# viridityzhu/HiFiHR

Measured on AMD Instinct MI355X. Metric: train images/sec, FreiHAND 224x224 (ResNet-18 + MANO LBS + render + losses + Adam), higher is better.
Workload: dtype f32; 1 GPU; BASELINE configs[1]: FreiHAND batch=32/GPU, ResNet-18 encoder + MANO LBS + silhouette/texture render losses, 224x224, aa=3 (672^2 samples); per_gpu_batch=32, global_batch=32, parallelism=dp1

## Files before the change

### hifihr_amd/_lib.py

```python
from __future__ import annotations

import ctypes
import os
from ctypes import POINTER, c_char_p, c_float, c_int, c_int32, c_long, c_size_t, c_void_p

import torch

_HERE = os.path.dirname(os.path.abspath(__file__))
LIB_PATH = os.path.join(_HERE, "libhifihr.so")

_c_float_p = POINTER(c_float)


class _LinearDesc(ctypes.Structure):
    _fields_ = [("x", c_void_p), ("w", c_void_p), ("b", c_void_p), ("y", c_void_p), ("B", c_int), ("I", c_int), ("O", c_int), ("act", c_int),
                ("dy", c_void_p), ("dz_scratch", c_void_p), ("dW_acc", c_void_p), ("db_acc", c_void_p), ("dx", c_void_p)]

_c_int_p = POINTER(c_int32)


class HifihrError(RuntimeError):
    pass


# ... 114 lines not shown
        c.hifihr_photo_loss_partial_floats.restype = c_int
        c.hifihr_photo_loss_fwd.argtypes = [_c_float_p, _c_float_p, c_void_p, c_int, c_int, c_int, c_float, c_float, c_float] + \
            [_c_float_p] * 4 + [c_void_p]
        c.hifihr_photo_loss_bwd.argtypes = [_c_float_p] * 6 + [c_int, c_int, c_int, c_float, c_float, _c_float_p, c_void_p]
        c.hifihr_sil_post.argtypes = [_c_float_p, _c_float_p, c_int, c_int, c_int, _c_float_p, _c_float_p, c_void_p]
        c.hifihr_linear_fwd.argtypes = [_c_float_p] * 3 + [c_int] * 4 + [_c_float_p] * 2 + [c_float, c_float] + [_c_float_p] * 6 + [c_void_p]
        c.hifihr_linear_bwd.argtypes = [_c_float_p] * 4 + [c_int] * 4 + [_c_float_p] * 10 + [c_void_p]
        c.hifihr_linear_fwd_group.argtypes = [POINTER(_LinearDesc), c_int, c_void_p]
        c.hifihr_linear_bwd_group.argtypes = [POINTER(_LinearDesc), c_int, c_void_p]
        c.hifihr_conv2d_bwd_data_pre.argtypes = [_c_float_p] * 3 + [c_int] * 9 + [c_void_p, c_size_t, c_void_p]
        c.hifihr_conv2d_bwd_data_pre_res.argtypes = [_c_float_p] * 4 + [c_int] * 9 + [c_void_p, c_size_t, c_void_p]
        c.hifihr_conv2d_bwd_data_pre_plus1x1.argtypes = [_c_float_p] * 5 + [c_int] * 9 + [c_void_p]
        c.hifihr_conv2d_bwd_data_pre_plus1x1_supported.argtypes = [c_int] * 9
        c.hifihr_conv2d_bwd_weight_plus1x1.argtypes = [_c_float_p] * 5 + [c_int] * 9 + [c_void_p]
        c.hifihr_conv2d_bwd_weight_plus1x1_supported.argtypes = [c_int] * 9
        c.hifihr_weight_prep.argtypes = [c_void_p, c_int, c_int, c_void_p]
        c.hifihr_freihand_augment.argtypes = [c_void_p, c_void_p, _c_int_p, _c_int_p, c_int, c_int, c_int, _c_float_p, _c_float_p, c_void_p]
        c.hifihr_ho3d_workspace_bytes.argtypes = [c_int, c_int]
        c.hifihr_ho3d_workspace_bytes.restype = c_size_t
        c.hifihr_ho3d_batch.argtypes = ([c_void_p, c_void_p] + [_c_float_p] * 3 + [c_int, c_int, _c_int_p, c_int, c_int, c_void_p, c_size_t] +
                                        [_c_float_p] * 5 + [c_void_p])
        c.hifihr_freihand_batch.argtypes = ([c_void_p, c_void_p] + [_c_float_p] * 4 + [c_int, c_int, _c_int_p, c_int, c_int, c_int, _c_float_p,
                                            _c_float_p, c_void_p] + [_c_float_p] * 6 + [c_void_p, c_void_p])
        c.hifihr_freihand_batch_step.argtypes = ([c_void_p, c_void_p] + [_c_float_p] * 4 + [c_int, c_int, _c_int_p, c_int, c_int, c_int, _c_float_p,
                                                 _c_float_p, c_void_p] + [_c_float_p] * 6 + [c_void_p, c_int, c_float] + [_c_float_p] * 4 + [c_void_p])
        c.hifihr_light_split_fwd.argtypes = [_c_float_p, c_int, _c_float_p, _c_float_p, c_void_p]
        c.hifihr_light_split_bwd.argtypes = [_c_float_p, _c_float_p, _c_float_p, c_int, _c_float_p, c_void_p]
        c.hifihr_wino4_bwd_gemm_pair_supported.argtypes = [c_int] * 5
        c.hifihr_wino4_bwd_gemm_pair.argtypes = [_c_float_p] * 6 + [c_int] * 6 + [c_void_p]
        c.hifihr_loss_total_fwd.argtypes = [POINTER(_c_float_p), POINTER(c_int), c_int, _c_float_p, c_void_p]
# ... 460 lines not shown
    def conv2d_bwd_data_pre_res(self, dy, wt, res, dx, N, H, W, C, K, R, S, stride, pad, ws=None):
        wsp, wsb = self._ws(ws)
        self.check(self.c.hifihr_conv2d_bwd_data_pre_res(_fp(dy), _fp(wt), _fp(res), _fp(dx), N, H, W, C, K, R, S, stride, pad, wsp, wsb,
                                                         _stream_of(dy)), "hifihr_conv2d_bwd_data_pre_res")

    def conv2d_bwd_data_pre_plus1x1_supported(self, N, H, W, C, K, R, S, stride, pad):
        return bool(self.c.hifihr_conv2d_bwd_data_pre_plus1x1_supported(int(N), int(H), int(W), int(C), int(K), int(R), int(S), int(stride), int(pad)))

    def conv2d_bwd_data_pre_plus1x1(self, dy, wt, dy2, wt2, dx, N, H, W, C, K, R, S, stride, pad):
        self.check(self.c.hifihr_conv2d_bwd_data_pre_plus1x1(_fp(dy), _fp(wt), _fp(dy2), _fp(wt2), _fp(dx), N, H, W, C, K, R, S, stride, pad,
                                                             _stream_of(dy)), "hifihr_conv2d_bwd_data_pre_plus1x1")

    def conv2d_bwd_weight_plus1x1_supported(self, N, H, W, C, K, R, S, stride, pad):
        return bool(self.c.hifihr_conv2d_bwd_weight_plus1x1_supported(int(N), int(H), int(W), int(C), int(K), int(R), int(S), int(stride), int(pad)))

    def conv2d_bwd_weight_plus1x1(self, x, dy, dw, dy2, dw2, N, H, W, C, K, R, S, stride, pad):
        self.check(self.c.hifihr_conv2d_bwd_weight_plus1x1(_fp(x), _fp(dy), _fp(dw), _fp(dy2), _fp(dw2), N, H, W, C, K, R, S, stride, pad,
                                                           _stream_of(x)), "hifihr_conv2d_bwd_weight_plus1x1")

    @staticmethod
    def prep_jobs(jobs, device):
        import struct
        raw = b"".join(struct.pack("<QQiiii", s.data_ptr(), d.data_ptr(), K, C, RS, kind) for s, d, K, C, RS, kind in jobs)
        return torch.frombuffer(bytearray(raw), dtype=torch.uint8).to(device)

    def weight_prep(self, table, njobs, blocks_per_job=64):
        self.check(self.c.hifihr_weight_prep(c_void_p(table.data_ptr()), njobs, blocks_per_job, _stream_of(table)), "hifihr_weight_prep")

    def freihand_batch(self, img_rgbx, mask, Ks, joints, verts, scales, packed, B, out, root_id=None, image_size=None):
        n, H, W = img_rgbx.shape
# ... 497 lines not shown
```

### hifihr_amd/csrc/conv.hip

```cpp
#include <hip/hip_runtime.h>

#include <cstdio>
#include <cstdlib>

#include "hifihr_internal.h"

namespace hifihr {

#if defined(HIFIHR_HOSTSIM)
typedef hs_floatx16 floatx16;
#else
typedef float floatx16 __attribute__((ext_vector_type(16)));
#endif

#if defined(HIFIHR_HOSTSIM)
#define HIFIHR_KEEP(x) ((void)0)
#define HIFIHR_SCHED_FENCE() ((void)0)
#else
#define HIFIHR_SCHED_FENCE() __builtin_amdgcn_sched_barrier(0)
#define HIFIHR_KEEP(x) asm volatile("" : "+v"(x))
#endif


struct SkArgs {
// ... 549 lines not shown
    __syncthreads();
  }
#pragma unroll
  for (int i = 0; i < TM; ++i)
#pragma unroll
    for (int j = 0; j < TN; ++j) {
      const int qq = bq0 + wn * (BN / 2) + j * 32 + r31;
#pragma unroll
      for (int e = 0; e < 16; ++e) {
        const int k = bk0 + wm * (BM / 2) + i * 32 + (e & 3) + 8 * (e >> 2) + 4 * half;
        if (k < K && qq < Q) atomicAdd(dw + (size_t)k * Q + qq, acc[i][j][e]);
      }
    }
}

__global__ __launch_bounds__(256) void weight_transpose_kernel(const float* __restrict__ w, float* __restrict__ wt, int K, int RS, int C) {
  const size_t n = (size_t)K * RS * C;
  for (size_t i = (size_t)blockIdx.x * 256 + threadIdx.x; i < n; i += (size_t)gridDim.x * 256) {
    const int k = (int)(i % K);
    const size_t rest = i / K;
    const int rs = (int)(rest % RS);
    const int c = (int)(rest / RS);
    wt[i] = w[((size_t)k * RS + rs) * C + c];
  }
}

__global__ __launch_bounds__(256) void image_to_nhwc4_kernel(const float* __restrict__ img, float4* __restrict__ out, int B, int H, int W,
                                                            int OH, int OW, int pt, int pl, int normalize) {
  const size_t n = (size_t)B * OH * OW, HW = (size_t)H * W;
  for (size_t i = (size_t)blockIdx.x * 256 + threadIdx.x; i < n; i += (size_t)gridDim.x * 256) {
// ... 403 lines not shown
  else snprintf(out, cap, "%s", kWgradKernelName[(int)k]);
}

bool conv_wgrad_plus1x1_supported(const ConvGeom& g) {
  static const int on = env_int("HIFIHR_WGRAD_PLUS1X1", 1);
  return on && !g.dgrad && g.stride >= 2 && g.pad < g.R && g.pad < g.S && g.batch <= 1 && g.IC % 4 == 0 && g.OC % 4 == 0 &&
         g.OH == (g.IH - 1) / g.stride + 1 && g.OW == (g.IW - 1) / g.stride + 1 && plan_wgrad(g, SIZE_MAX).kernel == WgradKernel::tiled;
}
hipError_t launch_conv_wgrad_plus1x1(const ConvGeom& g, const float* x, const float* dy, float* dw, const float* dy2, float* dw2, hipStream_t st) {
  if (!conv_wgrad_plus1x1_supported(g) || dy2 == nullptr || dw2 == nullptr) return hipErrorInvalidValue;
  const long M = (long)g.N * g.OH * g.OW;
  launch_wgrad_tile<64, 64, 16>(g, g.R * g.S * g.IC, M, device_cus() * 8, x, dy, dw, st, dy2, dw2);
  return hipGetLastError();
}

bool conv_wgrad_c3_supported(const ConvGeom& g) { return g.IC == 4 && conv_stem_wgrad_supported(g); }
hipError_t launch_conv_wgrad_c3(const ConvGeom& g, const float* x, const float* dy, float* dw3, void* ws, size_t ws_bytes, hipStream_t st) {
  if (!conv_wgrad_c3_supported(g) || ws == nullptr || ws_bytes < conv_stem_wgrad_slab_bytes()) return hipErrorInvalidValue;
  return launch_conv_stem_wgrad(g, x, dy, dw3, static_cast<float*>(ws), st, 3);
}

hipError_t launch_conv_wgrad(const ConvGeom& g, const float* x, const float* dy, float* dw, void* ws, size_t ws_bytes, hipStream_t st) {
  const long M = (long)g.N * g.OH * g.OW;
  const int Q = g.R * g.S * g.IC;
  if (g.IC % 4 != 0 || g.OC % 4 != 0) return hipErrorInvalidValue;
  const WgradPlan p = plan_wgrad(g, ws != nullptr ? ws_bytes : 0);
  float* slabs = ws_bytes >= p.ws_bytes ? static_cast<float*>(ws) : nullptr;
  hipError_t e = hipErrorNotReady;
  if (p.kernel == WgradKernel::gemm) {
    e = launch_bgemm_tn(dy, x, slabs, g.OC, g.IC, (int)M, 1, p.parts, st);
// ... 46 lines not shown
```

### hifihr_amd/csrc/gemm.hip

```cpp
#include <hip/hip_runtime.h>

#include <cstdio>
#include <cstdlib>
#include <type_traits>

#include "hifihr_internal.h"
#include "lds_dma.h"

namespace hifihr {

template <int BM, int BN>
__global__ __launch_bounds__(256) void bgemm_nt_kernel(BgemmArgs a) {
  constexpr int WM = BM / 2, WN = BN / 2;
  constexpr int TI = WN / 16, TJ = WM / 16;
  constexpr int STAGE = (BM + BN) * 32;
  constexpr int PA = BM / 32, PB = BN / 32;
  __shared__ __attribute__((aligned(1024))) float lds[2 * STAGE];
  const int tid = threadIdx.x, lane = tid & 63, wave = tid >> 6;
  const int wm = wave >> 1, wn = wave & 1;
  const int r = lane & 15, g = lane >> 4;

  int wg = xcd_remap((int)blockIdx.x, (int)gridDim.x);
  const int tiles_pb = a.tiles_m * a.tiles_n;
  const int p = wg / tiles_pb;
// ... 1316 lines not shown
  }
}

__global__ __launch_bounds__(512) void bgemm_tn_rows_kernel(BgemmArgs a, long per) {
  __shared__ __attribute__((aligned(1024))) float lds[4 * kRowsStage];
  tn_rows_body(a, per, lds, (int)blockIdx.x, (int)gridDim.x);
}

__global__ __launch_bounds__(512) void bgemm_nt_tn_pair_kernel(BgemmArgs a, long per_a, int ga, BgemmArgs b, long per_b) {
  __shared__ __attribute__((aligned(1024))) float lds[4 * kRowsStage];
  if ((int)blockIdx.x < ga) nt_rows_body<0>(a, per_a, lds, (int)blockIdx.x, ga);
  else tn_rows_body(b, per_b, lds, (int)blockIdx.x - ga, (int)gridDim.x - ga);
}

constexpr int kUnset = -(1 << 30);
static int gemm_cus() {
  const int v = env_int("HIFIHR_GEMM_CUS", 0);
  return v > 0 ? v : device_cus();
}
struct GemmEnv {
  int rows, tn_rows, tn_split, tn_coherent, tn_skip, pair, conv_rows, conv_rows_pair;
  int cus, loaders, sk, nt_tile, tn_tile, tn_parts;
  bool rows_on() const { return rows && nt_tile == kUnset; }
  bool tn_rows_on() const { return tn_rows && tn_tile == kUnset && tn_parts == kUnset; }
};
static GemmEnv gemm_env() {
  static const GemmEnv once = [] {
    GemmEnv e{};
    e.rows = env_int("HIFIHR_GEMM_ROWS", 1);
    e.tn_rows = env_int("HIFIHR_GEMM_TN_ROWS", 1); e.tn_split = env_int("HIFIHR_GEMM_TN_SPLIT", 1);
    e.tn_coherent = env_int("HIFIHR_GEMM_TN_COHERENT", 1); e.tn_skip = env_int("HIFIHR_GEMM_TN_SKIP", 1);
// ... 378 lines not shown
```

### hifihr_amd/csrc/hifihr_api.hip

```cpp
#include <hip/hip_runtime.h>

#include <algorithm>
#include <array>
#include <cmath>
#include <cstdarg>
#include <cstdio>
#include <cstring>
#include <new>
#include <vector>

#include "../../include/hifihr.h"
#include "hifihr_internal.h"
#include "mano_math.h"

namespace {

thread_local char g_err[512] = "";

int fail(int code, const char* fmt, ...) {
  va_list ap;
  va_start(ap, fmt);
  vsnprintf(g_err, sizeof(g_err), fmt, ap);
  va_end(ap);
  return code;
// ... 717 lines not shown
int hifihr_conv2d_bwd_weight_plus1x1_supported(int N, int H, int W, int C, int K, int R, int S, int stride, int pad) {
  if (!conv_dims_ok(N, H, W, C, K, R, S, stride, pad) || C % 4 || K % 4) return 0;
  const hifihr::ConvGeom g = conv_geom(N, H, W, C, K, R, S, stride, pad);
  return hifihr::conv_wgrad_plus1x1_supported(g) ? 1 : 0;
}

int hifihr_conv2d_bwd_weight_plus1x1(const float* x, const float* dy, float* dw, const float* dy2, float* dw2, int N, int H, int W, int C, int K,
                                     int R, int S, int stride, int pad, void* stream) {
  if (!x || !dy || !dw || !dy2 || !dw2 || !hifihr_conv2d_bwd_weight_plus1x1_supported(N, H, W, C, K, R, S, stride, pad))
    return fail(HIFIHR_EINVAL, "hifihr_conv2d_bwd_weight_plus1x1: bad argument (see hifihr_conv2d_bwd_weight_plus1x1_supported)");
  const hifihr::ConvGeom g = conv_geom(N, H, W, C, K, R, S, stride, pad);
  HIP_TRY(hifihr::launch_conv_wgrad_plus1x1(g, x, dy, dw, dy2, dw2, (hipStream_t)stream));
  return HIFIHR_OK;
}

int hifihr_weight_prep(const hifihr_prep_job* jobs, int njobs, int blocks_per_job, void* stream) {
  static_assert(sizeof(hifihr_prep_job) == sizeof(hifihr::PrepJob), "hifihr_prep_job layout");
  if (!jobs || njobs <= 0 || blocks_per_job <= 0) return fail(HIFIHR_EINVAL, "hifihr_weight_prep: bad argument");
  HIP_TRY(hifihr::launch_weight_prep(reinterpret_cast<const hifihr::PrepJob*>(jobs), njobs, blocks_per_job, (hipStream_t)stream));
  return HIFIHR_OK;
}

int hifihr_conv2d_bwd_weight(const float* x, const float* dy, float* dw, int N, int H, int W, int C, int K, int R, int S,
                             int stride, int pad, void* stream) {
  return hifihr_conv2d_bwd_weight_ws(x, dy, dw, N, H, W, C, K, R, S, stride, pad, nullptr, 0, stream);
}

size_t hifihr_conv2d_wgrad_workspace_bytes(int N, int H, int W, int C, int K, int R, int S, int stride, int pad) {
  if (!conv_dims_ok(N, H, W, C, K, R, S, stride, pad) || C % 4 || K % 4) return 0;
  const hifihr::ConvGeom g = conv_geom(N, H, W, C, K, R, S, stride, pad);
// ... 931 lines not shown
```

### hifihr_amd/csrc/hifihr_internal.h

```cpp
#pragma once
#include <hip/hip_runtime.h>

#include <cstdint>
#include <cstdlib>
#include <stdint.h>

#include "render_math.h"

namespace hifihr {

inline int device_cus() {
  static int cus = 0;
  if (cus == 0) {
    int dev = 0;
    hipDeviceProp_t prop;
    if (hipGetDevice(&dev) == hipSuccess && hipGetDeviceProperties(&prop, dev) == hipSuccess && prop.multiProcessorCount > 0) cus = prop.multiProcessorCount;
  }
  return cus > 0 ? cus : 256;
}

static inline int env_int(const char* name, int unset) {
  const char* e = getenv(name);
  return e ? atoi(e) : unset;
}
// ... 167 lines not shown
                             float* running_mean, float* running_var, hipStream_t st);
hipError_t launch_bn_act_eval(const float* x, const float* running_mean, const float* running_var, const float* gamma, const float* beta,
                              const float* residual, int act, long M, int C, float eps, float* y, hipStream_t st);
hipError_t launch_bn_act_bwd(const float* dy, const float* y, const float* x, const float* save_mean, const float* save_invstd,
                             const float* gamma, const float* beta, int act, long M, int C, float* red, float* dx, float* dres,
                             float* dgamma_acc, float* dbeta_acc, hipStream_t st);
bool bn_relu_maxpool_supported(int N, int H, int W, int C);
hipError_t launch_bn_relu_maxpool_fwd(const float* x, float* stats, const float* gamma, const float* beta, int N, int H, int W, int C,
                                      float eps, float momentum, float* y, unsigned char* tap, float* save_mean, float* save_invstd,
                                      float* running_mean, float* running_var, hipStream_t st);
hipError_t launch_bn_relu_maxpool_bwd(const float* gy, const unsigned char* tap, const float* x, const float* save_mean,
                                      const float* save_invstd, const float* gamma, const float* beta, int N, int H, int W, int C, float* red,
                                      float* dx, float* dgamma_acc, float* dbeta_acc, hipStream_t st, const float* pooled = nullptr);
size_t conv_wgrad_workspace_bytes(const ConvGeom& g);
hipError_t launch_conv_wgrad(const ConvGeom& g, const float* x, const float* dy, float* dw, void* ws, size_t ws_bytes, hipStream_t st);
bool conv_is_gemm(const ConvGeom& g);
bool conv_wgrad_c3_supported(const ConvGeom& g);
hipError_t launch_conv_wgrad_c3(const ConvGeom& g, const float* x, const float* dy, float* dw3, void* ws, size_t ws_bytes, hipStream_t st);
hipError_t launch_weight_transpose(const float* w, float* wt, int K, int RS, int C, hipStream_t st);
hipError_t launch_image_to_nhwc4(const float* img, float* out, int B, int H, int W, int OH, int OW, int pt, int pl, int normalize,
                                 hipStream_t st);

hipError_t launch_image_scale_to_nhwc4(const float* img, float* out, int B, int H, int W, const float* shift3, const float* scale3,
                                       hipStream_t st);
hipError_t launch_maxpool_notap(const float* x, int N, int H, int W, int C, int k, int s, int p, float* y, hipStream_t st);
int lpips_tap_max_channels();
size_t lpips_tap_partial_floats(int B);
hipError_t launch_lpips_tap(const float* f0, const float* f1, const float* w, int B, int HW, int C, int accumulate, float* partial, float* val,
                            hipStream_t st);

// ... 242 lines not shown
```

### hifihr_amd/ops.py

```python
from __future__ import annotations

import math
import os
import threading

import torch

from ._lib import get_lib, require_cuda


import os as _os

_DEBUG_SYNC = _os.environ.get("HIFIHR_DEBUG_SYNC", "0") == "1"


class _Profile:

    def __init__(self):
        self.on = False
        self.events = []
        self.last_render = None
        self.conv_log = []

    def enable(self):
# ... 635 lines not shown

    def end(self):
        self.active = False


_WEIGHT_PREP = _WeightPrep()


class _DeferredDw:

    def __init__(self):
        self.on = os.environ.get("HIFIHR_DEFER_DW", "1") != "0"
        self.active = False
        self.jobs = []
        self.halo = []
        self.pending = set()
        self.early = os.environ.get("HIFIHR_DEFER_EARLY", "1") != "0"
        self.side, self.home, self._streams, self.n_early = None, None, {}, 0

    def wants(self, w, direct):
        if self.side is not None and w.grad is not None and w.grad.data_ptr() in self.pending:
            torch.cuda.current_stream(self.side.device).wait_stream(self.side)
        return (self.on and self.active and direct and not _ASYNC_WGRAD.active and getattr(w, "_hifihr_grad_ready", None) is None
                and (w.grad is None or w.grad.data_ptr() not in self.pending))

    def add(self, dU, parts, tgt, K, C):
        self.jobs.append((dU, int(parts), tgt, int(K), int(C), torch.cuda.current_stream(tgt.device).cuda_stream))
        self.pending.add(tgt.data_ptr())

    def add_halo(self, slabs, nslab, tgt):
        self.halo.append((slabs, int(nslab), tgt, torch.cuda.current_stream(tgt.device).cuda_stream))
        self.pending.add(tgt.data_ptr())

    def clear(self):
        self.jobs.clear(); self.halo.clear(); self.pending.clear()
        if self.side is not None:
            if not torch.cuda.is_current_stream_capturing():
                torch.cuda.current_stream(self.side.device).wait_stream(self.side)
            self.side = None

    def _run(self, jobs, halo):
        lib = get_lib() if (jobs or halo) else None
        if halo:
            PROFILE.bracket("halo_reduce_multi", lambda: lib.conv_halo_wgrad_reduce_multi([h[:3] for h in halo]))
        if jobs:
            PROFILE.bracket("wino_dw_multi", lambda: lib.wino4_dw_transform_multi([j[:5] for j in jobs]))

    def flush(self):
        jobs, self.jobs = self.jobs, []
        halo, self.halo = self.halo, []
        self.pending.clear()
        self._run(jobs, halo)
        if self.side is not None:
            cur = torch.cuda.current_stream(self.side.device)
            cur.wait_stream(self.side)
            if self.home is not None and self.home != cur:
                self.home.wait_stream(self.side)
            self.side = None

    def flush_early(self, device):
        if not (self.early and self.active and self.side is None and (self.jobs or self.halo)):
            return
        cur = torch.cuda.current_stream(device)
        h = cur.cuda_stream
        jobs, halo = [j for j in self.jobs if j[5] == h], [j for j in self.halo if j[3] == h]
        if not (jobs or halo):
            return
        self.jobs, self.halo = [j for j in self.jobs if j[5] != h], [j for j in self.halo if j[3] != h]
        st = self._streams.get(device)
        if st is None:
            st = self._streams[device] = torch.cuda.Stream(device=device)
        st.wait_stream(cur)
        with torch.cuda.stream(st):
            self._run(jobs, halo)
        self.side, self.home, self.n_early = st, cur, self.n_early + 1


_DEFER_DW = _DeferredDw()


class _AsyncWgrad:

    def __init__(self):
        self.active, self.streams, self.refs = False, {}, []

    def stream(self, device):
        s = self.streams.get(device)
        if s is None:
            s = torch.cuda.Stream(device=device)
# ... 179 lines not shown
            PROFILE.bracket("conv_dgrad", lambda: lib.conv3x3_c64_wino(gy, U2, None, False, dx, None, N, H, W))
        return dx, None
    tgt, dw = _grad_target(w, wk, _CL)
    if PROFILE.on:
        PROFILE.conv_log.append((geom, "c64-pair"))
    nslab = lib.conv2d_wgrad_workspace_bytes(*geom)
    if nslab and dw is None and _DEFER_DW.wants(w, True):
        own = _wino_scratch(gy.device, ("c64slabs", w.data_ptr()), (nslab + 3) // 4)
        box = []
        PROFILE.bracket("conv_dgrad", lambda: box.append(lib.conv3x3_c64_bwd_pair_slabs(gy, U2, g_fork, dx, x, own, N, H, W)))
        _DEFER_DW.add_halo(own, box[-1], tgt)
    else:
        slabs = _wgrad_slabs(gy.device, nslab) if nslab else None
        PROFILE.bracket("conv_dgrad", lambda: lib.conv3x3_c64_bwd_pair(gy, U2, g_fork, dx, x, tgt, N, H, W, ws=slabs))
    return dx, dw


def _direct_dgrad(lib, gy, x, wk, w, geom, g_fork, plus1x1):
    dx = torch.empty_like(x, memory_format=_CL)
    ws = _conv_ws(lib, x.device, geom, True)
    if PROFILE.on:
        PROFILE.conv_log.append((geom, "dgrad" if plus1x1 is None else "dgrad+1x1"))
    wt = _WEIGHT_PREP.get(w, wk, 0)
    if plus1x1 is not None:
        assert wt is not None and g_fork is None
        PROFILE.bracket("conv_dgrad", lambda: lib.conv2d_bwd_data_pre_plus1x1(gy, wt, plus1x1[0], plus1x1[1], dx, *geom))
    elif wt is not None and g_fork is not None:
        PROFILE.bracket("conv_dgrad", lambda: lib.conv2d_bwd_data_pre_res(gy, wt, g_fork, dx, *geom, ws=ws))
    elif wt is not None:
        PROFILE.bracket("conv_dgrad", lambda: lib.conv2d_bwd_data_pre(gy, wt, dx, *geom, ws=ws))
# ... 52 lines not shown
            Yt = yt if yt is not None else _wino_scratch(dev, ("Yt", w.data_ptr()) if _ASYNC_WGRAD.active else "Yt", P * T * K)
            if slabs is None:
                slabs = _wino_wgrad_slabs(lib, w, dw is None, _ASYNC_WGRAD.active, dev, N, H, W, C, K, m)
            if PROFILE.on and not paired:
                PROFILE.conv_log.append((("wino", N, H, W, C, K, m), "gemm-tn"))

            def run_w():
                if yt is None:
                    lib.wino_dy_transform(gy, Yt, N, H, W, K, m)
                _wino_wgrad_tail(lib, v_saved, Yt, slabs, tgt, N, H, W, C, K, m, paired)
            go = lambda: PROFILE.bracket("conv_wgrad_wino", run_w)
            keep = (gy, v_saved, Yt, tgt)
        else:
            if PROFILE.on:
                PROFILE.conv_log.append((geom, "wgrad"))
            nslab = lib.conv2d_wgrad_workspace_bytes(*geom)
            go = lambda: PROFILE.bracket("conv_wgrad", lambda: lib.conv2d_bwd_weight(
                x, gy, tgt, *geom, ws=_wgrad_slabs(gy.device, nslab) if nslab else None))
            keep = (gy, x, tgt)
        if _ASYNC_WGRAD.active and dw is None:
            _ASYNC_WGRAD.launch(dev, go, keep)
        else:
            go()
        if dw is None:
            _grad_ready(w)
    if dx is None and g_fork is not None:
        dx = g_fork
    return dx, dw, db


class _Conv2dMFMA(torch.autograd.Function):
    @staticmethod
    def forward(ctx, x, w, stride, pad, want_stats=False, bias=None, relu=False, grad_premasked=False, mask_input_grad=False, fork=False):
# ... 126 lines not shown
            lib = get_lib()
            if lib.conv2d_bwd_data_pre_plus1x1_supported(N, H, W, C, K1, R, S, stride, pad):
                wt1, wt2 = _WEIGHT_PREP.get(ctx.w1, wk1, 0), _WEIGHT_PREP.get(ctx.w2, wk2, 0)
                if wt1 is not None and wt2 is not None:
                    plus = (gy2.contiguous(memory_format=_CL), wt2)
        if plus is not None:
            w_both = (need_w1 and need_w2 and not _ASYNC_WGRAD.active
                      and lib.conv2d_bwd_weight_plus1x1_supported(N, H, W, C, K1, R, S, stride, pad))
            dw1 = dw2 = None
            if w_both:
                gy1c = gy1.contiguous(memory_format=_CL)
                t1, dw1 = _grad_target(ctx.w1, wk1, _CL)
                t2, dw2 = _grad_target(ctx.w2, wk2, _CL)
                if PROFILE.on:
                    PROFILE.conv_log.append((ctx.geom1, "wgrad+1x1"))
                PROFILE.bracket("conv_wgrad", lambda: lib.conv2d_bwd_weight_plus1x1(x, gy1c, t1, plus[0], t2, N, H, W, C, K1, R, S, stride, pad))
                if dw1 is None:
                    _grad_ready(ctx.w1)
                if dw2 is None:
                    _grad_ready(ctx.w2)
            else:
                dw2 = conv(gy2, wk2, ctx.geom2, ctx.w2, False, need_w2)[1]
            dx, dw1b, _ = conv(gy1, wk1, ctx.geom1, ctx.w1, need_x, need_w1 and not w_both, plus1x1=plus)
            return dx, (dw1 if w_both else dw1b), dw2, None
        dx2 = dw2 = dw1 = None
        if gy2 is not None:
            dx2, dw2, _ = conv(gy2, wk2, ctx.geom2, ctx.w2, need_x, need_w2)
        if gy1 is not None:
            dx, dw1, _ = conv(gy1, wk1, ctx.geom1, ctx.w1, need_x, need_w1, g_fork=dx2)
        else:
            dx = dx2
# ... 1010 lines not shown
```

### include/hifihr.h

```cpp
#ifndef HIFIHR_H
#define HIFIHR_H

#include <stddef.h>
#include <stdint.h>

#ifdef __cplusplus
extern "C" {
#endif

#define HIFIHR_OK 0
#define HIFIHR_EINVAL (-1)
#define HIFIHR_EHIP (-2)
#define HIFIHR_ENOMEM (-3)

#define HIFIHR_MANO_NV 778
#define HIFIHR_MANO_NF 1538
#define HIFIHR_MANO_NJ 16

int hifihr_version(void);
const char* hifihr_last_error(void);
int hifihr_device_count(void);

typedef struct hifihr_mano hifihr_mano_t;

// ... 192 lines not shown
                    void* ws_d , size_t ws_bytes, void* stream);
int hifihr_bgemm_tn_parts(int M, int N, int T, int batch);
int hifihr_bgemm_describe(int tn, int M, int N, int K_or_T, int batch, char* out, int cap);
int hifihr_bgemm_tn(const float* a_d, const float* b_d, float* c_parts_d, int M, int N, int T, int batch, int parts, void* stream);
int hifihr_weight_transpose(const float* w_d, float* wt_d, int K, int RS, int C, void* stream);
int hifihr_conv2d_bwd_data_pre(const float* dy_d, const float* wt_d, float* dx_d, int N, int H, int W, int C, int K, int R, int S,
                               int stride, int pad, void* ws_d, size_t ws_bytes, void* stream);
int hifihr_conv2d_bwd_data_pre_res(const float* dy_d, const float* wt_d, const float* res_d, float* dx_d, int N, int H, int W, int C, int K,
                                   int R, int S, int stride, int pad, void* ws_d, size_t ws_bytes, void* stream);
int hifihr_conv2d_bwd_data_pre_plus1x1_supported(int N, int H, int W, int C, int K, int R, int S, int stride, int pad);
int hifihr_conv2d_bwd_data_pre_plus1x1(const float* dy_d, const float* wt_d, const float* dy2_d, const float* wt2_d, float* dx_d, int N, int H,
                                       int W, int C, int K, int R, int S, int stride, int pad, void* stream);
int hifihr_conv2d_bwd_weight_plus1x1_supported(int N, int H, int W, int C, int K, int R, int S, int stride, int pad);
int hifihr_conv2d_bwd_weight_plus1x1(const float* x_d, const float* dy_d, float* dw_d, const float* dy2_d, float* dw2_d, int N, int H, int W,
                                     int C, int K, int R, int S, int stride, int pad, void* stream);
typedef struct hifihr_prep_job {
  const float* src;
  float* dst;
  int K, C, RS, kind;
} hifihr_prep_job;
int hifihr_weight_prep(const hifihr_prep_job* jobs_d, int njobs, int blocks_per_job, void* stream);

int hifihr_conv2d_describe(int N, int H, int W, int C, int K, int R, int S, int stride, int pad, int direction, char* out, int cap);

int hifihr_conv2d_fwd_bnstats(const float* x_d, const float* w_d, float* y_d, float* stats_d, int N, int H, int W, int C, int K,
                              int R, int S, int stride, int pad, void* ws_d, size_t ws_bytes, void* stream);
int hifihr_conv2d_fwd_bnstats_pair_supported(int N, int H, int W, int C, int stride, int K1, int R1, int pad1, int K2, int R2, int pad2);
int hifihr_conv2d_fwd_bnstats_pair(const float* x_d, const float* w1_d, float* y1_d, float* stats1_d, int K1, int R1, int pad1, const float* w2_d,
                                   float* y2_d, float* stats2_d, int K2, int R2, int pad2, int N, int H, int W, int C, int stride, void* stream);

// ... 162 lines not shown
```

Baseline: 6716 images/sec.

## Split tiled conv wgrad over M into per-share slabs with deferred batched reduce

Adds a split-K style weight-gradient kernel for tiled convs. It partitions the reduction over N*OH*OW into shares sized to fill the CUs, and each workgroup writes a 64x64 partial tile to its own slab. A multi-job reduce kernel sums the slabs into dw, and the deferred-grad machinery can batch that reduce and run it on a side stream. The goal is more parallelism for wgrad GEMMs that have few output tiles. The cost is extra slab memory traffic, an added reduce launch, and more scratch buffers.

```diff
diff --git a/hifihr_amd/_lib.py b/hifihr_amd/_lib.py
--- a/hifihr_amd/_lib.py
+++ b/hifihr_amd/_lib.py
@@ -152,6 +152,11 @@
         c.hifihr_conv2d_bwd_data_pre_plus1x1_supported.argtypes = [c_int] * 9
         c.hifihr_conv2d_bwd_weight_plus1x1.argtypes = [_c_float_p] * 5 + [c_int] * 9 + [c_void_p]
         c.hifihr_conv2d_bwd_weight_plus1x1_supported.argtypes = [c_int] * 9
+        c.hifihr_conv2d_wgrad_slabs_bytes.argtypes = [c_int] * 10
+        c.hifihr_conv2d_wgrad_slabs_bytes.restype = c_size_t
+        c.hifihr_conv2d_bwd_weight_slabs.argtypes = [_c_float_p] * 3 + [c_int] * 9 + [c_void_p, c_size_t, c_void_p, c_void_p]
+        c.hifihr_conv2d_bwd_weight_plus1x1_slabs.argtypes = [_c_float_p] * 5 + [c_int] * 9 + [c_void_p, c_size_t, c_void_p, c_void_p]
+        c.hifihr_conv2d_wgrad_slabs_reduce_multi.argtypes = [c_void_p, c_int, c_void_p]
         c.hifihr_weight_prep.argtypes = [c_void_p, c_int, c_int, c_void_p]
         c.hifihr_freihand_augment.argtypes = [c_void_p, c_void_p, _c_int_p, _c_int_p, c_int, c_int, c_int, _c_float_p, _c_float_p, c_void_p]
         c.hifihr_ho3d_workspace_bytes.argtypes = [c_int, c_int]
@@ -642,6 +647,33 @@
     def conv2d_bwd_weight_plus1x1_supported(self, N, H, W, C, K, R, S, stride, pad):
         return bool(self.c.hifihr_conv2d_bwd_weight_plus1x1_supported(int(N), int(H), int(W), int(C), int(K), int(R), int(S), int(stride), int(pad)))
 
+    def conv2d_wgrad_slabs_bytes(self, N, H, W, C, K, R, S, stride, pad, plus1x1=False):
+        return int(self.c.hifihr_conv2d_wgrad_slabs_bytes(int(N), int(H), int(W), int(C), int(K), int(R), int(S), int(stride), int(pad), int(bool(plus1x1))))
+
+    def conv2d_bwd_weight_slabs(self, x, dy, dw, N, H, W, C, K, R, S, stride, pad, slabs, dy2=None, dw2=None, defer=False, slab_bytes=None):
+        import ctypes
+        n = ctypes.c_int(0)
+        np_ = ctypes.cast(ctypes.pointer(n), c_void_p) if defer else None
+        nb = 0 if slabs is None else slabs.numel() * slabs.element_size()
+        if slab_bytes is not None:
+            nb = min(nb, int(slab_bytes))
+        if dy2 is None:
+            self.check(self.c.hifihr_conv2d_bwd_weight_slabs(_fp(x), _fp(dy), _fp(dw), N, H, W, C, K, R, S, stride, pad, _fp(slabs), nb, np_,
+                                                             _stream_of(x)), "hifihr_conv2d_bwd_weight_slabs")
+        else:
+            self.check(self.c.hifihr_conv2d_bwd_weight_plus1x1_slabs(_fp(x), _fp(dy), _fp(dw), _fp(dy2), _fp(dw2), N, H, W, C, K, R, S, stride, pad,
+                                                                     _fp(slabs), nb, np_, _stream_of(x)), "hifihr_conv2d_bwd_weight_plus1x1_slabs")
+        return n.value
+
+    def conv2d_wgrad_slabs_reduce_multi(self, jobs):
+        import ctypes
+        import struct
+        raw = b"".join(struct.pack("<QQQiiii", sl.data_ptr(), dw.data_ptr(), 0 if dw2 is None else dw2.data_ptr(), int(n), int(K), int(Q), int(Q2))
+                       for sl, n, dw, dw2, K, Q, Q2 in jobs)
+        buf = ctypes.create_string_buffer(raw, len(raw))
+        self.check(self.c.hifihr_conv2d_wgrad_slabs_reduce_multi(ctypes.cast(buf, c_void_p), len(jobs), _stream_of(jobs[0][0])),
+                   "hifihr_conv2d_wgrad_slabs_reduce_multi")
+
     def conv2d_bwd_weight_plus1x1(self, x, dy, dw, dy2, dw2, N, H, W, C, K, R, S, stride, pad):
         self.check(self.c.hifihr_conv2d_bwd_weight_plus1x1(_fp(x), _fp(dy), _fp(dw), _fp(dy2), _fp(dw2), N, H, W, C, K, R, S, stride, pad,
                                                            _stream_of(x)), "hifihr_conv2d_bwd_weight_plus1x1")
diff --git a/hifihr_amd/csrc/conv.hip b/hifihr_amd/csrc/conv.hip
--- a/hifihr_amd/csrc/conv.hip
+++ b/hifihr_amd/csrc/conv.hip
@@ -587,6 +587,169 @@
     }
 }
 
+constexpr int kWgradSlabBK = 32;
+constexpr int kWgradSlabWgsPerCu = 3;
+constexpr int kWgradSlabTile = 64 * 64;
+struct WgradSlabArgs {
+  const float *x, *dy, *dy2;
+  float* slabs;
+  int qtiles1, qtiles, tiles, cps;
+  int dn, doh, dow;
+};
+
+template <int BKW>
+__global__ __launch_bounds__(256) void conv_wgrad_slab_kernel(ConvGeom g, WgradSlabArgs a) {
+  constexpr int BM = 64, BN = 64;
+  constexpr int LA = BM + 4, LB = BN + 4;
+  __shared__ __attribute__((aligned(16))) float As[2][BKW * LA];
+  __shared__ __attribute__((aligned(16))) float Bs[2][BKW * LB];
+  const int tid = threadIdx.x, lane = tid & 63, wave = tid >> 6;
+  const int wm = wave >> 1, wn = wave & 1;
+  const int half = lane >> 5, r31 = lane & 31;
+  const int M = g.N * g.OH * g.OW;
+  const int b = (int)blockIdx.x;
+  const int share = b / a.tiles, tile = b - share * a.tiles;
+  const int kt = tile / a.qtiles, qt = tile - kt * a.qtiles;
+  const bool second = qt >= a.qtiles1;
+  const float* __restrict__ x = a.x;
+  const float* __restrict__ dy = second ? a.dy2 : a.dy;
+  const int Q = second ? g.IC : g.R * g.S * g.IC;
+  const int K = g.OC;
+  const int bq0 = (second ? qt - a.qtiles1 : qt) * BN, bk0 = kt * BM;
+  const int nch_total = (M + BKW - 1) / BKW;
+  const int ch_lo = share * a.cps;
+  const int ch_hi = min(ch_lo + a.cps, nch_total);
+
+  constexpr int APR = BM / 4, BPR = BN / 4;
+  constexpr int AROWS = 256 / APR, BROWS = 256 / BPR;
+  constexpr int AL = BKW / AROWS, BL = BKW / BROWS;
+  const int a_row = tid / APR, a_col = (tid % APR) * 4;
+  const int b_row = tid / BPR, b_col = (tid % BPR) * 4;
+  const int q = bq0 + b_col;
+  const bool qok = q < Q;
+  int qr = 0, qs = 0, qc = 0;
+  if (qok && second) {
+    qc = q; qr = g.pad; qs = g.pad;
+  } else if (qok) {
+    const int t = q / g.IC;
+    qc = q - t * g.IC;
+    qr = t / g.S;
+    qs = t - qr * g.S;
+  }
+  int pn[BL], poh[BL], pow_[BL];
+#pragma unroll
+  for (int i = 0; i < BL; ++i) {
+    const int m = ch_lo * BKW + b_row + BROWS * i;
+    pn[i] = m / (g.OH * g.OW);
+    const int rem = m - pn[i] * (g.OH * g.OW);
+    poh[i] = rem / g.OW;
+    pow_[i] = rem - poh[i] * g.OW;
+  }
+  float4 ra[AL], rb[BL];
+  bool va[AL], vb[BL];
+  auto load_global = [&](int ch) {
+    const int m0 = ch * BKW;
+    const bool chok = ch < ch_hi;
+#pragma unroll
+    for (int i = 0; i < AL; ++i) {
+      const int m = m0 + a_row + AROWS * i;
+      const int k = bk0 + a_col;
+      const bool ok = chok && m < M && k < K;
+      ra[i] = *reinterpret_cast<const float4*>(dy + (ok ? (size_t)m * K + k : 0));
+      va[i] = ok;
+    }
+#pragma unroll
+    for (int i = 0; i < BL; ++i) {
+      const int m = m0 + b_row + BROWS * i;
+      const int n = pn[i], oh = poh[i], ow = pow_[i];
+      pow_[i] += a.dow;
+      const int c1 = pow_[i] >= g.OW;
+      pow_[i] -= c1 ? g.OW : 0;
+      poh[i] += a.doh + c1;
+      const int c2 = poh[i] >= g.OH;
+      poh[i] -= c2 ? g.OH : 0;
+      pn[i] += a.dn + c2;
+      const int ih = oh * g.stride - g.pad + qr, iw = ow * g.stride - g.pad + qs;
+      const bool ok = chok && m < M && qok && ih >= 0 && ih < g.IH && iw >= 0 && iw < g.IW;
+      rb[i] = *reinterpret_cast<const float4*>(x + (ok ? (((size_t)n * g.IH + ih) * g.IW + iw) * g.IC + qc : 0));
+      vb[i] = ok;
+    }
+  };
+  auto store_lds = [&](int buf) {
+#pragma unroll
+    for (int i = 0; i < AL; ++i)
+      *reinterpret_cast<float4*>(&As[buf][(a_row + AROWS * i) * LA + a_col]) = va[i] ? ra[i] : make_float4(0.f, 0.f, 0.f, 0.f);
+#pragma unroll
+    for (int i = 0; i < BL; ++i)
+      *reinterpret_cast<float4*>(&Bs[buf][(b_row + BROWS * i) * LB + b_col]) = vb[i] ? rb[i] : make_float4(0.f, 0.f, 0.f, 0.f);
+  };
+
+  floatx16 acc;
+#pragma unroll
+  for (int e = 0; e < 16; ++e) acc[e] = 0.f;
+
+  load_global(ch_lo);
+  store_lds(0);
+  __syncthreads();
+  for (int ch = ch_lo; ch < ch_hi; ++ch) {
+    const int buf = (ch - ch_lo) & 1;
+    load_global(ch + 1);
+    HIFIHR_SCHED_FENCE();
+#pragma unroll
+    for (int t = 0; t < BKW / 2; ++t) {
+      const float av = As[buf][(2 * t + half) * LA + wm * (BM / 2) + r31];
+      const float bv = Bs[buf][(2 * t + half) * LB + wn * (BN / 2) + r31];
+      acc = __builtin_amdgcn_mfma_f32_32x32x2f32(av, bv, acc, 0, 0, 0);
+    }
+    HIFIHR_SCHED_FENCE();
+    store_lds(buf ^ 1);
+    __syncthreads();
+  }
+  float4* sl = reinterpret_cast<float4*>(a.slabs) + ((size_t)share * a.tiles + tile) * (kWgradSlabTile / 4);
+#pragma unroll
+  for (int e4 = 0; e4 < 4; ++e4) sl[e4 * 256 + tid] = make_float4(acc[4 * e4], acc[4 * e4 + 1], acc[4 * e4 + 2], acc[4 * e4 + 3]);
+}
+
+constexpr int kWgradSlabMaxJobs = 16;
+struct WgradSlabJobs {
+  const float* slabs[kWgradSlabMaxJobs];
+  float* dw[kWgradSlabMaxJobs];
+  float* dw2[kWgradSlabMaxJobs];
+  int nshare[kWgradSlabMaxJobs], K[kWgradSlabMaxJobs], Q[kWgradSlabMaxJobs], Q2[kWgradSlabMaxJobs];
+};
+__global__ __launch_bounds__(256) void conv_wgrad_slab_reduce_kernel(WgradSlabJobs js) {
+  const int j = blockIdx.y;
+  const int K = js.K[j], Q1 = js.Q[j], Q2 = js.Q2[j];
+  const int qtiles1 = (Q1 + 63) / 64, qtiles = qtiles1 + (Q2 + 63) / 64, tiles = ((K + 63) / 64) * qtiles;
+  const int tile = (int)blockIdx.x >> 2, e4 = (int)blockIdx.x & 3;
+  if (tile >= tiles) return;
+  const int tid = threadIdx.x, lane = tid & 63, wave = tid >> 6;
+  const int wm = wave >> 1, wn = wave & 1, half = lane >> 5, r31 = lane & 31;
+  const float4* __restrict__ sl = reinterpret_cast<const float4*>(js.slabs[j]) + (size_t)tile * (kWgradSlabTile / 4) + e4 * 256 + tid;
+  const size_t share_stride = (size_t)tiles * (kWgradSlabTile / 4);
+  const int nshare = js.nshare[j];
+  float4 s = make_float4(0.f, 0.f, 0.f, 0.f);
+  for (int z0 = 0; z0 < nshare; z0 += 8) {
+    float4 v[8];
+#pragma unroll
+    for (int u = 0; u < 8; ++u) v[u] = (z0 + u < nshare) ? sl[(size_t)(z0 + u) * share_stride] : make_float4(0.f, 0.f, 0.f, 0.f);
+#pragma unroll
+    for (int u = 0; u < 8; ++u) { s.x += v[u].x; s.y += v[u].y; s.z += v[u].z; s.w += v[u].w; }
+  }
+  const int kt = tile / qtiles, qt = tile - kt * qtiles;
+  const bool second = qt >= qtiles1;
+  float* __restrict__ dw = second ? js.dw2[j] : js.dw[j];
+  const int Q = second ? Q2 : Q1;
+  const int qq = (second ? qt - qtiles1 : qt) * 64 + wn * 32 + r31;
+  const int k0 = kt * 64 + wm * 32 + 8 * e4 + 4 * half;
+  if (qq < Q) {
+    const float sv[4] = {s.x, s.y, s.z, s.w};
+#pragma unroll
+    for (int c = 0; c < 4; ++c)
+      if (k0 + c < K) dw[(size_t)(k0 + c) * Q + qq] += sv[c];
+  }
+}
+
 __global__ __launch_bounds__(256) void weight_transpose_kernel(const float* __restrict__ w, float* __restrict__ wt, int K, int RS, int C) {
   const size_t n = (size_t)K * RS * C;
   for (size_t i = (size_t)blockIdx.x * 256 + threadIdx.x; i < n; i += (size_t)gridDim.x * 256) {
@@ -1020,6 +1183,78 @@
   return hipGetLastError();
 }
 
+struct WgradSlabPlan {
+  bool ok;
+  int qtiles1, qtiles2, ktiles, tiles, shares, cps;
+  size_t bytes;
+};
+static WgradSlabPlan plan_wgrad_slabs(const ConvGeom& g, bool plus1x1) {
+  WgradSlabPlan p{};
+  const long M = (long)g.N * g.OH * g.OW;
+  if (g.dgrad || g.batch > 1 || g.IC % 4 != 0 || g.OC % 4 != 0 || M <= 0 || M >= (1L << 30)) return p;
+  const WgradPlan w = plan_wgrad(g, SIZE_MAX);
+  if (w.kernel != WgradKernel::tiled || w.bm != 64) return p;
+  if (plus1x1 && !conv_wgrad_plus1x1_supported(g)) return p;
+  p.qtiles1 = (g.R * g.S * g.IC + 63) / 64;
+  p.qtiles2 = plus1x1 ? (g.IC + 63) / 64 : 0;
+  p.ktiles = (g.OC + 63) / 64;
+  const long tiles = (long)p.ktiles * (p.qtiles1 + p.qtiles2);
+  if (tiles >= (1L << 20)) return p;
+  p.tiles = (int)tiles;
+  const int nch = (int)((M + kWgradSlabBK - 1) / kWgradSlabBK);
+  int shares = gemm_cus() * kWgradSlabWgsPerCu / p.tiles;
+  if (shares > nch / 4) shares = nch / 4;
+  if (shares < 1) shares = 1;
+  p.cps = (nch + shares - 1) / shares;
+  p.shares = (nch + p.cps - 1) / p.cps;
+  p.bytes = (size_t)p.shares * p.tiles * kWgradSlabTile * sizeof(float);
+  p.ok = true;
+  return p;
+}
+size_t conv_wgrad_slabs_bytes(const ConvGeom& g, bool plus1x1) { return plan_wgrad_slabs(g, plus1x1).bytes; }
+
+hipError_t launch_conv_wgrad_slab_reduce_multi(const WgradSlabJob* jobs, int njobs, hipStream_t st) {
+  for (int base = 0; base < njobs; base += kWgradSlabMaxJobs) {
+    WgradSlabJobs js;
+    const int n = njobs - base < kWgradSlabMaxJobs ? njobs - base : kWgradSlabMaxJobs;
+    int widest = 0;
+    for (int q = 0; q < n; ++q) {
+      const WgradSlabJob& j = jobs[base + q];
+      if (j.slabs == nullptr || j.dw == nullptr || j.nshare <= 0 || j.K <= 0 || j.Q <= 0 || j.Q2 < 0 || (j.Q2 > 0 && j.dw2 == nullptr)) return hipErrorInvalidValue;
+      js.slabs[q] = j.slabs; js.dw[q] = j.dw; js.dw2[q] = j.dw2; js.nshare[q] = j.nshare; js.K[q] = j.K; js.Q[q] = j.Q; js.Q2[q] = j.Q2;
+      const long tiles = (long)((j.K + 63) / 64) * ((j.Q + 63) / 64 + (j.Q2 + 63) / 64);
+      if (tiles >= (1L << 20)) return hipErrorInvalidValue;
+      if ((int)tiles > widest) widest = (int)tiles;
+    }
+    hipLaunchKernelGGL(conv_wgrad_slab_reduce_kernel, dim3(widest * 4, n), dim3(256), 0, st, js);
+  }
+  return hipGetLastError();
+}
+
+hipError_t launch_conv_wgrad_slabs(const ConvGeom& g, const float* x, const float* dy, float* dw, const float* dy2, float* dw2, void* slabs,
+                                   size_t slab_bytes, int* nshare_out, hipStream_t st) {
+  const bool plus = dy2 != nullptr;
+  if (plus != (dw2 != nullptr) || g.IC % 4 != 0 || g.OC % 4 != 0) return hipErrorInvalidValue;
+  if (plus && !conv_wgrad_plus1x1_supported(g)) return hipErrorInvalidValue;
+  const WgradSlabPlan p = plan_wgrad_slabs(g, plus);
+  if (nshare_out != nullptr) *nshare_out = 0;
+  if (!p.ok || slabs == nullptr || slab_bytes < p.bytes) {
+    if (plus) return launch_conv_wgrad_plus1x1(g, x, dy, dw, dy2, dw2, st);
+    return launch_conv_wgrad(g, x, dy, dw, nullptr, 0, st);
+  }
+  WgradSlabArgs a;
+  a.x = x; a.dy = dy; a.dy2 = dy2; a.slabs = static_cast<float*>(slabs);
+  a.qtiles1 = p.qtiles1; a.qtiles = p.qtiles1 + p.qtiles2; a.tiles = p.tiles; a.cps = p.cps;
+  const int plane = g.OH * g.OW;
+  a.dn = kWgradSlabBK / plane;
+  a.doh = (kWgradSlabBK - a.dn * plane) / g.OW;
+  a.dow = kWgradSlabBK - a.dn * plane - a.doh * g.OW;
+  hipLaunchKernelGGL((conv_wgrad_slab_kernel<kWgradSlabBK>), dim3((unsigned)(p.tiles * p.shares)), dim3(256), 0, st, g, a);
+  if (nshare_out != nullptr) { *nshare_out = p.shares; return hipGetLastError(); }
+  const WgradSlabJob job{a.slabs, dw, dw2, p.shares, g.OC, g.R * g.S * g.IC, plus ? g.IC : 0};
+  return launch_conv_wgrad_slab_reduce_multi(&job, 1, st);
+}
+
 bool conv_wgrad_c3_supported(const ConvGeom& g) { return g.IC == 4 && conv_stem_wgrad_supported(g); }
 hipError_t launch_conv_wgrad_c3(const ConvGeom& g, const float* x, const float* dy, float* dw3, void* ws, size_t ws_bytes, hipStream_t st) {
   if (!conv_wgrad_c3_supported(g) || ws == nullptr || ws_bytes < conv_stem_wgrad_slab_bytes()) return hipErrorInvalidValue;
diff --git a/hifihr_amd/csrc/gemm.hip b/hifihr_amd/csrc/gemm.hip
--- a/hifihr_amd/csrc/gemm.hip
+++ b/hifihr_amd/csrc/gemm.hip
@@ -1354,7 +1354,7 @@
 }
 
 constexpr int kUnset = -(1 << 30);
-static int gemm_cus() {
+int gemm_cus() {
   const int v = env_int("HIFIHR_GEMM_CUS", 0);
   return v > 0 ? v : device_cus();
 }
diff --git a/hifihr_amd/csrc/hifihr_api.hip b/hifihr_amd/csrc/hifihr_api.hip
--- a/hifihr_amd/csrc/hifihr_api.hip
+++ b/hifihr_amd/csrc/hifihr_api.hip
@@ -755,6 +755,41 @@
   return HIFIHR_OK;
 }
 
+size_t hifihr_conv2d_wgrad_slabs_bytes(int N, int H, int W, int C, int K, int R, int S, int stride, int pad, int plus1x1) {
+  if (!conv_dims_ok(N, H, W, C, K, R, S, stride, pad) || C % 4 || K % 4) return 0;
+  const hifihr::ConvGeom g = conv_geom(N, H, W, C, K, R, S, stride, pad);
+  return hifihr::conv_wgrad_slabs_bytes(g, plus1x1 != 0);
+}
+
+int hifihr_conv2d_bwd_weight_slabs(const float* x, const float* dy, float* dw, int N, int H, int W, int C, int K, int R, int S, int stride, int pad,
+                                   void* slabs, size_t slab_bytes, int* nshare, void* stream) {
+  if (!x || !dy || !dw || !conv_dims_ok(N, H, W, C, K, R, S, stride, pad) || C % 4 || K % 4)
+    return fail(HIFIHR_EINVAL, "hifihr_conv2d_bwd_weight_slabs: bad argument (C and K must be multiples of 4)");
+  const hifihr::ConvGeom g = conv_geom(N, H, W, C, K, R, S, stride, pad);
+  HIP_TRY(hifihr::launch_conv_wgrad_slabs(g, x, dy, dw, nullptr, nullptr, slabs, slabs ? slab_bytes : 0, nshare, (hipStream_t)stream));
+  return HIFIHR_OK;
+}
+
+int hifihr_conv2d_bwd_weight_plus1x1_slabs(const float* x, const float* dy, float* dw, const float* dy2, float* dw2, int N, int H, int W, int C,
+                                           int K, int R, int S, int stride, int pad, void* slabs, size_t slab_bytes, int* nshare, void* stream) {
+  if (!x || !dy || !dw || !dy2 || !dw2 || !hifihr_conv2d_bwd_weight_plus1x1_supported(N, H, W, C, K, R, S, stride, pad))
+    return fail(HIFIHR_EINVAL, "hifihr_conv2d_bwd_weight_plus1x1_slabs: bad argument (see hifihr_conv2d_bwd_weight_plus1x1_supported)");
+  const hifihr::ConvGeom g = conv_geom(N, H, W, C, K, R, S, stride, pad);
+  HIP_TRY(hifihr::launch_conv_wgrad_slabs(g, x, dy, dw, dy2, dw2, slabs, slabs ? slab_bytes : 0, nshare, (hipStream_t)stream));
+  return HIFIHR_OK;
+}
+
+int hifihr_conv2d_wgrad_slabs_reduce_multi(const hifihr_wgrad_slab_job* jobs, int njobs, void* stream) {
+  static_assert(sizeof(hifihr_wgrad_slab_job) == sizeof(hifihr::WgradSlabJob), "job layouts");
+  if (!jobs || njobs <= 0) return fail(HIFIHR_EINVAL, "hifihr_conv2d_wgrad_slabs_reduce_multi: bad argument");
+  for (int i = 0; i < njobs; ++i)
+    if (!jobs[i].slabs_d || !jobs[i].dw_acc_d || jobs[i].nshare <= 0 || jobs[i].K <= 0 || jobs[i].Q <= 0 || jobs[i].Q2 < 0 ||
+        (jobs[i].Q2 > 0 && !jobs[i].dw2_acc_d))
+      return fail(HIFIHR_EINVAL, "hifihr_conv2d_wgrad_slabs_reduce_multi: bad job");
+  HIP_TRY(hifihr::launch_conv_wgrad_slab_reduce_multi(reinterpret_cast<const hifihr::WgradSlabJob*>(jobs), njobs, (hipStream_t)stream));
+  return HIFIHR_OK;
+}
+
 int hifihr_weight_prep(const hifihr_prep_job* jobs, int njobs, int blocks_per_job, void* stream) {
   static_assert(sizeof(hifihr_prep_job) == sizeof(hifihr::PrepJob), "hifihr_prep_job layout");
   if (!jobs || njobs <= 0 || blocks_per_job <= 0) return fail(HIFIHR_EINVAL, "hifihr_weight_prep: bad argument");
diff --git a/hifihr_amd/csrc/hifihr_internal.h b/hifihr_amd/csrc/hifihr_internal.h
--- a/hifihr_amd/csrc/hifihr_internal.h
+++ b/hifihr_amd/csrc/hifihr_internal.h
@@ -205,6 +205,12 @@
                                       float* dx, float* dgamma_acc, float* dbeta_acc, hipStream_t st, const float* pooled = nullptr);
 size_t conv_wgrad_workspace_bytes(const ConvGeom& g);
 hipError_t launch_conv_wgrad(const ConvGeom& g, const float* x, const float* dy, float* dw, void* ws, size_t ws_bytes, hipStream_t st);
+struct WgradSlabJob { const float* slabs; float* dw; float* dw2; int nshare, K, Q, Q2; };
+size_t conv_wgrad_slabs_bytes(const ConvGeom& g, bool plus1x1);
+hipError_t launch_conv_wgrad_slabs(const ConvGeom& g, const float* x, const float* dy, float* dw, const float* dy2, float* dw2, void* slabs,
+                                   size_t slab_bytes, int* nshare_out, hipStream_t st);
+hipError_t launch_conv_wgrad_slab_reduce_multi(const WgradSlabJob* jobs, int njobs, hipStream_t st);
+int gemm_cus();
 bool conv_is_gemm(const ConvGeom& g);
 bool conv_wgrad_c3_supported(const ConvGeom& g);
 hipError_t launch_conv_wgrad_c3(const ConvGeom& g, const float* x, const float* dy, float* dw3, void* ws, size_t ws_bytes, hipStream_t st);
diff --git a/hifihr_amd/ops.py b/hifihr_amd/ops.py
--- a/hifihr_amd/ops.py
+++ b/hifihr_amd/ops.py
@@ -673,6 +673,7 @@
         self.active = False
         self.jobs = []
         self.halo = []
+        self.slab = []
         self.pending = set()
         self.early = os.environ.get("HIFIHR_DEFER_EARLY", "1") != "0"
         self.side, self.home, self._streams, self.n_early = None, None, {}, 0
@@ -691,15 +692,23 @@
         self.halo.append((slabs, int(nslab), tgt, torch.cuda.current_stream(tgt.device).cuda_stream))
         self.pending.add(tgt.data_ptr())
 
+    def add_slab(self, slabs, nshare, tgt, tgt2, K, Q, Q2):
+        self.slab.append((slabs, int(nshare), tgt, tgt2, int(K), int(Q), int(Q2), torch.cuda.current_stream(tgt.device).cuda_stream))
+        self.pending.add(tgt.data_ptr())
+        if tgt2 is not None:
+            self.pending.add(tgt2.data_ptr())
+
     def clear(self):
-        self.jobs.clear(); self.halo.clear(); self.pending.clear()
+        self.jobs.clear(); self.halo.clear(); self.slab.clear(); self.pending.clear()
         if self.side is not None:
             if not torch.cuda.is_current_stream_capturing():
                 torch.cuda.current_stream(self.side.device).wait_stream(self.side)
             self.side = None
 
-    def _run(self, jobs, halo):
-        lib = get_lib() if (jobs or halo) else None
+    def _run(self, jobs, halo, slab=()):
+        lib = get_lib() if (jobs or halo or slab) else None
+        if slab:
+            PROFILE.bracket("wgrad_slab_reduce_multi", lambda: lib.conv2d_wgrad_slabs_reduce_multi([j[:7] for j in slab]))
         if halo:
             PROFILE.bracket("halo_reduce_multi", lambda: lib.conv_halo_wgrad_reduce_multi([h[:3] for h in halo]))
         if jobs:
@@ -708,8 +717,9 @@
     def flush(self):
         jobs, self.jobs = self.jobs, []
         halo, self.halo = self.halo, []
+        slab, self.slab = self.slab, []
         self.pending.clear()
-        self._run(jobs, halo)
+        self._run(jobs, halo, slab)
         if self.side is not None:
             cur = torch.cuda.current_stream(self.side.device)
             cur.wait_stream(self.side)
@@ -718,20 +728,21 @@
             self.side = None
 
     def flush_early(self, device):
-        if not (self.early and self.active and self.side is None and (self.jobs or self.halo)):
+        if not (self.early and self.active and self.side is None and (self.jobs or self.halo or self.slab)):
             return
         cur = torch.cuda.current_stream(device)
         h = cur.cuda_stream
-        jobs, halo = [j for j in self.jobs if j[5] == h], [j for j in self.halo if j[3] == h]
-        if not (jobs or halo):
+        jobs, halo, slab = [j for j in self.jobs if j[5] == h], [j for j in self.halo if j[3] == h], [j for j in self.slab if j[7] == h]
+        if not (jobs or halo or slab):
             return
         self.jobs, self.halo = [j for j in self.jobs if j[5] != h], [j for j in self.halo if j[3] != h]
+        self.slab = [j for j in self.slab if j[7] != h]
         st = self._streams.get(device)
         if st is None:
             st = self._streams[device] = torch.cuda.Stream(device=device)
         st.wait_stream(cur)
         with torch.cuda.stream(st):
-            self._run(jobs, halo)
+            self._run(jobs, halo, slab)
         self.side, self.home, self.n_early = st, cur, self.n_early + 1
 
 
@@ -941,6 +952,24 @@
         slabs = _wgrad_slabs(gy.device, nslab) if nslab else None
         PROFILE.bracket("conv_dgrad", lambda: lib.conv3x3_c64_bwd_pair(gy, U2, g_fork, dx, x, tgt, N, H, W, ws=slabs))
     return dx, dw
+
+
+def _tiled_wgrad(lib, x, gy, tgt, geom, w, direct, gy2=None, tgt2=None, w2=None):
+    N, H, W, C, K, R, S, stride, pad = geom
+    nb = lib.conv2d_wgrad_slabs_bytes(*geom, gy2 is not None)
+    on_branch = torch.cuda.current_stream(gy.device).cuda_stream in BRANCH_STREAMS
+    if nb and direct and not on_branch and _DEFER_DW.wants(w, True) and (w2 is None or _DEFER_DW.wants(w2, True)):
+        own = _wino_scratch(gy.device, ("wgrad_slabs", w.data_ptr()), (nb + 3) // 4)
+        n = lib.conv2d_bwd_weight_slabs(x, gy, tgt, *geom, own, dy2=gy2, dw2=tgt2, defer=True)
+        if n:
+            _DEFER_DW.add_slab(own, n, tgt, tgt2, K, R * S * C, C if gy2 is not None else 0)
+    elif nb:
+        lib.conv2d_bwd_weight_slabs(x, gy, tgt, *geom, _wgrad_slabs(gy.device, nb), dy2=gy2, dw2=tgt2)
+    elif gy2 is not None:
+        lib.conv2d_bwd_weight_plus1x1(x, gy, tgt, gy2, tgt2, *geom)
+    else:
+        nslab = lib.conv2d_wgrad_workspace_bytes(*geom)
+        lib.conv2d_bwd_weight(x, gy, tgt, *geom, ws=_wgrad_slabs(gy.device, nslab) if nslab else None)
 
 
 def _direct_dgrad(lib, gy, x, wk, w, geom, g_fork, plus1x1):
@@ -1023,9 +1052,7 @@
         else:
             if PROFILE.on:
                 PROFILE.conv_log.append((geom, "wgrad"))
-            nslab = lib.conv2d_wgrad_workspace_bytes(*geom)
-            go = lambda: PROFILE.bracket("conv_wgrad", lambda: lib.conv2d_bwd_weight(
-                x, gy, tgt, *geom, ws=_wgrad_slabs(gy.device, nslab) if nslab else None))
+            go = lambda: PROFILE.bracket("conv_wgrad", lambda: _tiled_wgrad(lib, x, gy, tgt, geom, w, dw is None))
             keep = (gy, x, tgt)
         if _ASYNC_WGRAD.active and dw is None:
             _ASYNC_WGRAD.launch(dev, go, keep)
@@ -1182,7 +1209,8 @@
                 t2, dw2 = _grad_target(ctx.w2, wk2, _CL)
                 if PROFILE.on:
                     PROFILE.conv_log.append((ctx.geom1, "wgrad+1x1"))
-                PROFILE.bracket("conv_wgrad", lambda: lib.conv2d_bwd_weight_plus1x1(x, gy1c, t1, plus[0], t2, N, H, W, C, K1, R, S, stride, pad))
+                PROFILE.bracket("conv_wgrad", lambda: _tiled_wgrad(lib, x, gy1c, t1, ctx.geom1, ctx.w1, dw1 is None and dw2 is None,
+                                                                   gy2=plus[0], tgt2=t2, w2=ctx.w2))
                 if dw1 is None:
                     _grad_ready(ctx.w1)
                 if dw2 is None:
diff --git a/include/hifihr.h b/include/hifihr.h
--- a/include/hifihr.h
+++ b/include/hifihr.h
@@ -230,6 +230,19 @@
 int hifihr_conv2d_bwd_weight_plus1x1_supported(int N, int H, int W, int C, int K, int R, int S, int stride, int pad);
 int hifihr_conv2d_bwd_weight_plus1x1(const float* x_d, const float* dy_d, float* dw_d, const float* dy2_d, float* dw2_d, int N, int H, int W,
                                      int C, int K, int R, int S, int stride, int pad, void* stream);
+size_t hifihr_conv2d_wgrad_slabs_bytes(int N, int H, int W, int C, int K, int R, int S, int stride, int pad, int plus1x1);
+int hifihr_conv2d_bwd_weight_slabs(const float* x_d, const float* dy_d, float* dw_d, int N, int H, int W, int C, int K, int R, int S, int stride,
+                                   int pad, void* slabs_d, size_t slab_bytes, int* nshare , void* stream);
+int hifihr_conv2d_bwd_weight_plus1x1_slabs(const float* x_d, const float* dy_d, float* dw_d, const float* dy2_d, float* dw2_d, int N, int H, int W,
+                                           int C, int K, int R, int S, int stride, int pad, void* slabs_d, size_t slab_bytes,
+                                           int* nshare , void* stream);
+typedef struct hifihr_wgrad_slab_job {
+  const float* slabs_d;
+  float* dw_acc_d;
+  float* dw2_acc_d;
+  int nshare, K, Q, Q2;
+} hifihr_wgrad_slab_job;
+int hifihr_conv2d_wgrad_slabs_reduce_multi(const hifihr_wgrad_slab_job* jobs , int njobs, void* stream);
 typedef struct hifihr_prep_job {
   const float* src;
   float* dst;
```

Measured after the change: 6695 images/sec. No clear change (-0.3%).
